# jkk-research/urban_road_filter

Measured on NVIDIA H100. Metric: scans_per_sec, higher is better.
Workload: dtype f32/f64

## Files before the change

### urban_road_filter_b200/csrc/urf_kernels.cuh

```cuda
#pragma once
#include <type_traits>

#include "urf_device.cuh"
#include "urf_logic.cuh"
#include "urf_lomuto.cuh"
#include "urf_stdsort.cuh"
#include "urf_workspace.cuh"

namespace urf {

__constant__ float c_beam_d[kSectKeys];
__constant__ float c_beam_o[kSectKeys];
__constant__ unsigned char c_beam_yx[kSectKeys];

__device__ __forceinline__ int lane_id() { return threadIdx.x & 31; }
__device__ __forceinline__ unsigned scan_base(int b, int S) { return (unsigned)b * point_slice((unsigned)S); }

template <int N, class T>
__device__ __forceinline__ void warp_inclusive_sum(T (&x)[N]) {
#pragma unroll
  for (int d = 1; d < 32; d <<= 1) {
    T u[N];
#pragma unroll
    for (int i = 0; i < N; i++) u[i] = __shfl_up_sync(0xffffffffu, x[i], d);
// ... 181 lines not shown
        buf.sect[g] = (short)sec;
      }
      const unsigned peers = __match_any_sync(0xffffffffu, sec);
      if (sec >= 0 && lane_id() == __ffs(peers) - 1) atomicAdd(&s_scnt[sec], __popc(peers));
    }
#pragma unroll
    for (int j = 0; j < kPtsPerThread; ++j) cur[j] = nxt[j];
  }
  roi = __reduce_add_sync(0xffffffffu, roi);
  if (lane_id() == 0 && roi) atomicAdd(&s_roi, roi);
  __syncthreads();
  unsigned* fi = buf.firstidx + (size_t)b * kElevSlice;
  for (int e = threadIdx.x; e <= kElevBins; e += kPtsThreads) {
    const unsigned v = s_first[e];
    if (v != 0xffffffffu) atomicMin(&fi[e], v);
  }
  for (int s = threadIdx.x; s < kSectKeys; s += kPtsThreads)
    if (s_scnt[s]) atomicAdd(&buf.tab[b].sect_cnt[s], s_scnt[s]);
  if (threadIdx.x == 0 && s_roi) atomicAdd(&buf.out[b].n_roi, s_roi);
}

__device__ void register_exact_cta(const float* __restrict__ alpha, int n, float interval, int channels, float* s_vis,
                                   float* s_reg, int* s_idx, int* out_m) {
  int m = 0, vis = 0, i_last = -1;
  bool frozen = false;
  while (m < channels) {
    int local = 0x7fffffff;
    for (int i = i_last + 1 + threadIdx.x; i < n; i += blockDim.x) {
      const float a = alpha[i];
      if (a < 0.0f) continue;
      bool cov = false;
      for (int t = 0; t < vis; t++) {
        if (fabsf(__fsub_rn(s_vis[t], a)) <= interval) { cov = true; break; }
      }
      if (!cov) { local = i; break; }
    }
    const int istar = CtaGroup::min(local);
    if (istar == 0x7fffffff) break;
    const float a = alpha[istar];
    if (threadIdx.x == 0) { s_reg[m] = a; s_idx[m] = istar; if (!frozen && a != 0.0f) s_vis[vis] = a; }
    if (!frozen) { if (a == 0.0f) frozen = true; else vis++; }
    m++;
    i_last = istar;
    __syncthreads();
  }
  *out_m = m;
}

__device__ void publish_rings_cta(ScanTab& tab, ScanOut& out, unsigned short* lut, float interval, const float* s_reg,
                                  const int* s_idx, int m, unsigned long long* s_keys, float* s_sorted) {
  for (int t = threadIdx.x; t < kRingKeys; t += blockDim.x)
    s_keys[t] = t < m ? (((unsigned long long)fbits(s_reg[t]) << 32) | (unsigned)s_idx[t]) : ~0ull;
  __syncthreads();
  group_bitonic<CtaGroup>(s_keys, kRingKeys);
  for (int t = threadIdx.x; t < kRingKeys; t += blockDim.x) {
    if (t < m) {
      const float a = bitsf((unsigned)(s_keys[t] >> 32));
      s_sorted[t] = a;
      tab.angle[t] = a;
      tab.regidx[t] = (int)(unsigned)s_keys[t];
      tab.regorder[t] = s_idx[t];
    } else { s_sorted[t] = 0.f; tab.angle[t] = 0.f; tab.regidx[t] = 0x7fffffff; tab.regorder[t] = 0x7fffffff; }
  }
  if (threadIdx.x == 0) out.n_rings = m;
  __syncthreads();
  for (int e = threadIdx.x; e <= kElevBins; e += blockDim.x) lut[e] = (unsigned short)ring_lut_entry(s_sorted, m, interval, e);
}

__global__ void __launch_bounds__(256) k_register(DevBuffers buf, DevParams prm, int S) {
  const int b = blockIdx.x;
  const int n = buf.n[b];
  ScanOut& out = buf.out[b];
  ScanTab& tab = buf.tab[b];
  const float* alpha = buf.alpha_v + (size_t)b * point_slice(S);
  __shared__ unsigned s_cand[kMaxCand];
  __shared__ float s_calpha[kMaxCand];
  __shared__ float s_vis[kRingKeys];
  __shared__ float s_reg[kRingKeys];
  __shared__ float s_sorted[kRingKeys];
  __shared__ int s_idx[kRingKeys];
  __shared__ unsigned long long s_keys[kRingKeys];
  __shared__ int s_cnt, s_m;
  if (out.n_roi < 30) {
    if (threadIdx.x == 0) out.n_rings = 0;
    return;
  }
  bool exact = prm.force_exact || (out.flags & F_ZERO_ALPHA);
  if (!exact) {
    if (threadIdx.x == 0) s_cnt = 0;
    __syncthreads();
    const unsigned* fi = buf.firstidx + (size_t)b * kElevSlice;
    for (int t = threadIdx.x; t <= kElevBins; t += blockDim.x) {
      const unsigned v = fi[t];
      if (v != 0xffffffffu) { int s = atomicAdd(&s_cnt, 1); if (s < kMaxCand) s_cand[s] = v; }
    }
    __syncthreads();
    const int cnt = s_cnt;
    if (cnt > kMaxCand) exact = true;
    else {
      const int npad = next_pow2(cnt < 2 ? 2 : cnt);
      for (int t = cnt + threadIdx.x; t < npad; t += blockDim.x) s_cand[t] = 0xffffffffu;
      __syncthreads();
      group_bitonic<CtaGroup>(s_cand, npad);
      for (int t = threadIdx.x; t < cnt; t += blockDim.x) s_calpha[t] = alpha[s_cand[t]];
      __syncthreads();
      if (threadIdx.x < 32) {
        int m = 0;
        for (int c = 0; c < cnt && m < prm.channels; c++) {
          const float a = s_calpha[c];
          bool cov = false;
          for (int t = lane_id(); t < m; t += 32)
            if (fabsf(__fsub_rn(s_reg[t], a)) <= prm.interval) cov = true;
          cov = __any_sync(0xffffffffu, cov);
          if (!cov) {
            if (lane_id() == 0) { s_reg[m] = a; s_idx[m] = (int)s_cand[c]; }
            m++;
            __syncwarp();
          }
        }
        if (lane_id() == 0) s_m = m;
      }
      __syncthreads();
    }
  }
  if (exact) {
    int m;
    register_exact_cta(alpha, n, prm.interval, prm.channels, s_vis, s_reg, s_idx, &m);
    if (threadIdx.x == 0) { s_m = m; atomicOr(&out.flags, F_EXACT_REG); }
    __syncthreads();
  }
  publish_rings_cta(tab, out, buf.lut + (size_t)b * kElevSlice, prm.interval, s_reg, s_idx, s_m, s_keys, s_sorted);
}

__device__ __forceinline__ bool assign_chunk(const DevBuffers& buf, const DevParams& prm, int b, int S, int T, int chunk, int n, bool live,
                                             bool verify, const float* s_angle, const int* s_regidx, const int* regorder, int R,
                                             const unsigned short* __restrict__ lut, unsigned* cnt, int lane) {
  bool violation = false;
  constexpr int H = 8;
  static_assert((kChunk / 32) % H == 0, "chunk iterations come in groups of H");
#pragma unroll 1
  for (int h0 = 0; h0 < kChunk / 32; h0 += H) {
    float av[H];
    unsigned short start[H];
#pragma unroll
    for (int u = 0; u < H; u++) {
      const int i = chunk * kChunk + (h0 + u) * 32 + lane;
      av[u] = i < n ? buf.alpha_v[scan_base(b, S) + (unsigned)i] : -1.0f;
    }
#pragma unroll
    for (int u = 0; u < H; u++) start[u] = (live && av[u] >= 0.0f) ? lut[elev_bin(av[u])] : (unsigned short)0;
#pragma unroll
    for (int u = 0; u < H; u++) {
      const int i = chunk * kChunk + (h0 + u) * 32 + lane;
      int ring = -1;
      if (i < n) {
        const float a = av[u];
        const bool kept = live && a >= 0.0f;
        if (kept) {
          int lo;
          ring = assign_ring_from(s_angle, R, a, prm.interval, start[u], &lo);
          if (verify && registration_violation(s_angle, s_regidx, regorder, R, prm.channels, prm.interval, a, i, lo)) violation = true;
        }
        buf.ringid[scan_base(b, S) + (unsigned)i] = kept ? (short)ring : (short)-2;
      }
      const int ring0 = __shfl_sync(0xffffffffu, ring, 0);
      if (__all_sync(0xffffffffu, ring == ring0)) { if (lane == 0 && ring0 >= 0) atomicAdd(&cnt[ring0], 32u); }
      else if (ring >= 0) atomicAdd(&cnt[ring], 1u);
    }
  }
  __syncwarp();
  const int C = prm.channels;
  unsigned* row = buf.hist + ((size_t)b * chunk_rows(T) + chunk) * C;
  for (int t = lane; t < C; t += 32) row[t] = cnt[t];
  return violation;
}

__global__ void __launch_bounds__(kWarpsPerBlock * 32) k_assign(DevBuffers buf, DevParams prm, int S, int T) {
  const int b = blockIdx.y;
  ScanOut& out = buf.out[b];
  const int flags = out.flags;
  const int n = buf.n[b];
  const int warp = threadIdx.x >> 5, lane = lane_id();
  const int chunk = blockIdx.x * kWarpsPerBlock + warp;
  __shared__ float s_angle[kRingKeys];
  __shared__ int s_regidx[kRingKeys];
  __shared__ unsigned s_cnt[kWarpsPerBlock][kRingKeys];
  ScanTab& tab = buf.tab[b];
  const int R = out.n_rings;
  for (int t = threadIdx.x; t < kRingKeys; t += blockDim.x) { s_angle[t] = tab.angle[t]; s_regidx[t] = tab.regidx[t]; }
  for (int t = lane; t < kRingKeys; t += 32) s_cnt[warp][t] = 0;
  __syncthreads();
  if (chunk * kChunk >= n) return;
  const bool violation = assign_chunk(buf, prm, b, S, T, chunk, n, out.n_roi >= 30, !(flags & F_EXACT_REG), s_angle, s_regidx, tab.regorder, R,
                                      buf.lut + (size_t)b * kElevSlice, s_cnt[warp], lane);
  if (__any_sync(0xffffffffu, violation) && lane == 0) atomicOr(&out.flags, F_SPEC_VIOLATION);
}

constexpr int kScanOffThreads = 512, kScanOffWarps = kScanOffThreads / 32;
constexpr int kScanOffBatch = 16;
static_assert(kRingKeys < kScanOffThreads && kSectKeys <= kScanOffThreads, "one ring_start entry and one sector per thread");
__global__ void __launch_bounds__(kScanOffThreads, 2) k_scan_offsets(DevBuffers buf, DevParams prm, int S, int T) {
  __shared__ unsigned s_part[kScanOffWarps][kRingKeys];
  __shared__ unsigned s_base[kRingKeys];
  const int b = blockIdx.x;
  const int n = buf.n[b];
  const int C = prm.channels;
  const int rows = (n + kChunk - 1) / kChunk;
  const int warp = threadIdx.x >> 5, lane = lane_id();
  {
    ScanOut& out = buf.out[b];
    const int flags = out.flags;
    if ((flags & F_SPEC_VIOLATION) && !(flags & F_EXACT_REG)) {
      __shared__ float s_vis[kRingKeys], s_reg[kRingKeys], s_sorted[kRingKeys];
      __shared__ int s_idx[kRingKeys];
      __shared__ unsigned long long s_keys[kRingKeys];
      __shared__ int s_m;
      int m;
      register_exact_cta(buf.alpha_v + (size_t)b * point_slice(S), n, prm.interval, prm.channels, s_vis, s_reg, s_idx, &m);
      if (threadIdx.x == 0) s_m = m;
      __syncthreads();
      const unsigned short* lut = buf.lut + (size_t)b * kElevSlice;
      publish_rings_cta(buf.tab[b], out, buf.lut + (size_t)b * kElevSlice, prm.interval, s_reg, s_idx, s_m, s_keys, s_sorted);
      __syncthreads();
      const int R = s_m;
      for (int c0 = 0; c0 < rows; c0 += kScanOffWarps) {
        for (int t = lane; t < kRingKeys; t += 32) s_part[warp][t] = 0;
        __syncwarp();
        if (c0 + warp < rows) assign_chunk(buf, prm, b, S, T, c0 + warp, n, true, false, s_sorted, nullptr, nullptr, R, lut, s_part[warp], lane);
        __syncwarp();
      }
      if (threadIdx.x == 0) out.flags = flags | F_EXACT_REG;
      __syncthreads();
    }
  }
  ScanTab& tab = buf.tab[b];
  const unsigned scnt = threadIdx.x < kSectKeys ? (unsigned)tab.sect_cnt[threadIdx.x] : 0u;
  const int rpw = (rows + kScanOffWarps - 1) / kScanOffWarps;
  const int r0 = min(rows, warp * rpw), r1 = min(rows, (warp + 1) * rpw);
  unsigned* hist = buf.hist + (size_t)b * chunk_rows(T) * C;
  for (int key = lane; key < C; key += 32) {
    unsigned s = 0;
    for (int r = r0; r < r1; r += kScanOffBatch) {
      unsigned v[kScanOffBatch];
#pragma unroll
      for (int u = 0; u < kScanOffBatch; u++) v[u] = r + u < r1 ? hist[(size_t)(r + u) * C + key] : 0u;
#pragma unroll
      for (int u = 0; u < kScanOffBatch; u++) s += v[u];
    }
    s_part[warp][key] = s;
  }
  __syncthreads();
  unsigned rtot = 0;
  if (threadIdx.x < C)
    for (int w = 0; w < kScanOffWarps; w++) { const unsigned v = s_part[w][threadIdx.x]; s_part[w][threadIdx.x] = rtot; rtot += v; }
  unsigned x[2] = {rtot, scnt}, all[2];
  CtaGroup::exclusive_sum(x, all);
  const unsigned xr = x[0], xs = x[1], all_r = all[0], all_s = all[1];
  ScanOut& o = buf.out[b];
  if (threadIdx.x < C) s_base[threadIdx.x] = xr;
  if (threadIdx.x <= kRingKeys) o.ring_start[threadIdx.x] = (int)(threadIdx.x < C ? xr : all_r);
  if (threadIdx.x < kSectKeys) { tab.sect_start[threadIdx.x] = (int)xs; tab.sect_cur[threadIdx.x] = (int)xs; }
  if (threadIdx.x == 0) { o.n_order = (int)all_r; tab.sect_start[kSectKeys] = (int)all_s; }
  __syncthreads();
  for (int key = lane; key < C; key += 32) {
    unsigned run = s_base[key] + s_part[warp][key];
    for (int r = r0; r < r1; r += kScanOffBatch) {
      unsigned v[kScanOffBatch];
#pragma unroll
      for (int u = 0; u < kScanOffBatch; u++) v[u] = r + u < r1 ? hist[(size_t)(r + u) * C + key] : 0u;
#pragma unroll
      for (int u = 0; u < kScanOffBatch; u++)
        if (r + u < r1) { hist[(size_t)(r + u) * C + key] = run; run += v[u]; }
    }
  }
}

__device__ __forceinline__ void mbar_init(unsigned long long* bar, unsigned count) {
  asm volatile("mbarrier.init.shared::cta.b64 [%0], %1;\n" ::"r"((unsigned)__cvta_generic_to_shared(bar)), "r"(count) : "memory");
  asm volatile("fence.proxy.async.shared::cta;\n" ::: "memory");
}
__device__ __forceinline__ void bulk_copy_g2s(void* dst, const void* src, unsigned bytes, unsigned long long* bar) {
  const unsigned d = (unsigned)__cvta_generic_to_shared(dst), m = (unsigned)__cvta_generic_to_shared(bar);
  asm volatile("mbarrier.arrive.expect_tx.shared::cta.b64 _, [%0], %1;\n" ::"r"(m), "r"(bytes) : "memory");
  asm volatile("cp.async.bulk.shared::cluster.global.mbarrier::complete_tx::bytes [%0], [%1], %2, [%3];\n"
               ::"r"(d), "l"(src), "r"(bytes), "r"(m) : "memory");
}
__device__ __forceinline__ void mbar_wait(unsigned long long* bar, unsigned phase) {
  const unsigned m = (unsigned)__cvta_generic_to_shared(bar);
  unsigned done;
  do {
    asm volatile("{\n .reg .pred p;\n mbarrier.try_wait.parity.shared::cta.b64 p, [%1], %2;\n selp.u32 %0, 1, 0, p;\n}\n"
                 : "=r"(done) : "r"(m), "r"(phase) : "memory");
  } while (!done);
}
constexpr int kScatterWarps = 4;
constexpr size_t kScatterSmem = (size_t)kScatterWarps * kChunk * sizeof(float4);
__global__ void __launch_bounds__(kScatterWarps * 32, 4) k_scatter(DevBuffers buf, DevParams prm, int S, int T) {
  const int b = blockIdx.y;
  const int n = buf.n[b];
  const int warp = threadIdx.x >> 5, lane = lane_id();
  const int chunk = blockIdx.x * kScatterWarps + warp;
  extern __shared__ float4 s_tiles[];
  __shared__ unsigned long long s_bar[kScatterWarps];
  __shared__ unsigned s_delta[kScatterWarps][kChunk];
  __shared__ unsigned s_lcnt[kScatterWarps][kRingKeys];
  __shared__ unsigned short s_perm[kScatterWarps][kChunk];
  __shared__ int s_scnt[kSectKeys], s_sbase[kSectKeys];
  const float4* tile = s_tiles + warp * kChunk;
  unsigned* delta = s_delta[warp];
  unsigned* lcnt = s_lcnt[warp];
  unsigned short* perm = s_perm[warp];
  ScanTab& tab = buf.tab[b];
  const bool live = chunk * kChunk < n;
  const unsigned* row = buf.hist + ((size_t)b * chunk_rows(T) + chunk) * prm.channels;
  const unsigned gb = scan_base(b, S), g0 = gb + (unsigned)chunk * kChunk;
  if (live && lane == 0) {
    mbar_init(&s_bar[warp], 1);
    bulk_copy_g2s(s_tiles + warp * kChunk, buf.in + g0, (unsigned)min(kChunk, n - chunk * kChunk) * sizeof(float4), &s_bar[warp]);
  }
  for (int t = threadIdx.x; t < kSectKeys; t += blockDim.x) s_scnt[t] = 0;
  for (int t = lane; t < kRingKeys; t += 32) lcnt[t] = 0;
  __syncthreads();
  const unsigned lt = (1u << lane) - 1u;
  unsigned packed[kChunk / 32];
  unsigned spack[kChunk / 32];
  if (live) {
    constexpr int GRP = kChunk / 32;
#pragma unroll
    for (int h = 0; h < kChunk / 32 / GRP; h++) {
      short rr[GRP], ss[GRP];
#pragma unroll
      for (int u = 0; u < GRP; u++) {
        const int li = (h * GRP + u) * 32 + lane;
        const bool in = chunk * kChunk + li < n;
        rr[u] = in ? buf.ringid[g0 + li] : (short)-1;
        ss[u] = in ? buf.sect[g0 + li] : (short)-1;
      }
#pragma unroll
      for (int u = 0; u < GRP; u++) {
        const int it = h * GRP + u;
        const int sec = ss[u];
        const int sec0 = __shfl_sync(0xffffffffu, sec, 0);
        int srank = 0;
        if (__all_sync(0xffffffffu, sec == sec0)) {
          int sb = 0;
          if (lane == 0 && sec0 >= 0) sb = atomicAdd(&s_scnt[sec0], 32);
          srank = __shfl_sync(0xffffffffu, sb, 0) + lane;
        } else if (sec >= 0) srank = atomicAdd(&s_scnt[sec], 1);
        spack[it] = sec >= 0 ? (((unsigned)(sec + 1) << 16) | (unsigned)srank) : 0u;
        const int ring = rr[u];
        const int rprev = __shfl_up_sync(0xffffffffu, ring, 1), ring0 = __shfl_sync(0xffffffffu, ring, 0);
        unsigned peers;
        if (__all_sync(0xffffffffu, ring == ring0)) peers = 0xffffffffu;
        else if (__all_sync(0xffffffffu, lane == 0 || ring > rprev) || __all_sync(0xffffffffu, lane == 0 || ring < rprev)) peers = 1u << lane;
        else peers = __match_any_sync(0xffffffffu, ring);
        const int leader = __ffs(peers) - 1;
        unsigned rb = 0;
        if (ring >= 0 && lane == leader) rb = atomicAdd(&lcnt[ring], (unsigned)__popc(peers));
        rb = __shfl_sync(0xffffffffu, rb, leader);
        packed[it] = ring >= 0 ? (((unsigned)(ring + 1) << 16) | (rb + __popc(peers & lt))) : 0u;
      }
    }
  }
  __syncthreads();
  for (int t = threadIdx.x; t < kSectKeys; t += blockDim.x) {
    const int c = s_scnt[t];
    s_sbase[t] = c > 0 ? atomicAdd(&tab.sect_cur[t], c) : 0;
  }
  int total = 0;
  if (live) {
    {
      unsigned v[kRingKeys / 32], sum = 0;
#pragma unroll
      for (int j = 0; j < kRingKeys / 32; j++) { v[j] = lcnt[lane * (kRingKeys / 32) + j]; sum += v[j]; }
      unsigned inc[1] = {sum};
      warp_inclusive_sum(inc);
      unsigned run = inc[0] - sum;
      __syncwarp();
#pragma unroll
      for (int j = 0; j < kRingKeys / 32; j++) { lcnt[lane * (kRingKeys / 32) + j] = run; run += v[j]; }
    }
    __syncwarp();
#pragma unroll
    for (int it = 0; it < kChunk / 32; it++) {
      const unsigned pk = packed[it];
      if (pk) {
        const int ring = (int)(pk >> 16) - 1;
        const unsigned lstart = lcnt[ring];
        const int slot = lstart + (pk & 0xffffu);
        perm[slot] = (unsigned short)(it * 32 + lane);
        delta[slot] = __ldg(&row[ring]) - lstart;
      }
      total += __popc(__ballot_sync(0xffffffffu, pk != 0));
    }
    __syncwarp();
    mbar_wait(&s_bar[warp], 0);
    for (int t = lane; t < total; t += 32) {
      const int li = perm[t];
      const float4 p = tile[li];
      const unsigned dst = gb + delta[t] + (unsigned)t;
      buf.bpt[dst] = make_float4(p.x, p.y, p.z, __int_as_float(chunk * kChunk + li));
      if (prm.want_order) buf.baz[dst] = make_uint2(fbits(buf.az[g0 + li]), (unsigned)(chunk * kChunk + li));
    }
  }
  __syncthreads();
  if (live) {
#pragma unroll
    for (int it = 0; it < kChunk / 32; it++) {
      const unsigned sp = spack[it];
      if (sp) {
        const int sec = (int)(sp >> 16) - 1;
        const int li = it * 32 + lane;
        const float4 p = tile[li];
        const unsigned dst = gb + (unsigned)(s_sbase[sec] + (int)(sp & 0xffffu));
        buf.sr[dst] = star_radius(p.x, p.y);
        buf.sz[dst] = p.z;
        buf.sidx[dst] = (unsigned)(chunk * kChunk + li);
      }
    }
  }
}

constexpr int kWarpCap = 1024, kCtaCap = 8192;
constexpr int kNetCap = 512;
constexpr unsigned kSslIndex = 0x80000000u;

struct SectorRecs {
  const DevBuffers& buf;
  unsigned o;
  unsigned at;
  __device__ __forceinline__ const float* r() const { return buf.sr + o; }
  __device__ __forceinline__ unsigned key(int e) const { return fbits(buf.sr[o + (unsigned)e]); }
  __device__ __forceinline__ void put(int e, unsigned k, unsigned slot) const {
    buf.ssrz[at + (unsigned)e] = make_float2(bitsf(k), buf.sz[o + slot]);
    buf.ssl[at + (unsigned)e] = slot;
  }
};
__device__ __forceinline__ SectorRecs sector_recs(const DevBuffers& buf, int b, int S, int base, int at = 0) {
  const unsigned o = scan_base(b, S) + (unsigned)base;
  return SectorRecs{buf, o, o + (unsigned)at};
}
__device__ __forceinline__ int star_input_index(const DevBuffers& buf, unsigned o, int e) {
  const unsigned l = buf.ssl[o + (unsigned)e];
  return (l & kSslIndex) ? (int)(l & ~kSslIndex) : (int)buf.sidx[o + l];
}

template <int EPL, int WARPS, bool LIST = false, bool STAGED = false>
__device__ __forceinline__ bool bitonic_sector(const SectorRecs& d, int n, int tid, unsigned* s_xk, unsigned* s_xe) {
  constexpr int THREADS = WARPS * 32;
  const int lane = tid & 31;
  unsigned key[EPL], el[EPL];
#pragma unroll
  for (int r = 0; r < EPL; r++) {
    const int e = tid * EPL + r;
    key[r] = 0xffffffffu; el[r] = 0u;
    if (e < n) {
      if (LIST) { key[r] = s_xk[e]; el[r] = (STAGED && s_xe == nullptr) ? (unsigned)e : s_xe[e]; }
      else { key[r] = d.key(e); el[r] = (unsigned)e; }
    }
  }
  auto intra = [&](int k_over_epl, auto kc) {
    constexpr int K = decltype(kc)::value;
#pragma unroll
    for (int j = (K > 0 ? K : EPL) >> 1; j > 0; j >>= 1) {
#pragma unroll
      for (int r = 0; r < EPL; r++) {
        if ((r & j) == 0) {
          const bool asc = K > 0 ? ((r & K) == 0) : ((tid & k_over_epl) == 0);
          const bool sw = (key[r] > key[r | j]) == asc;
          const unsigned ka = sw ? key[r | j] : key[r], kb = sw ? key[r] : key[r | j];
          const unsigned ea = sw ? el[r | j] : el[r], eb = sw ? el[r] : el[r | j];
          key[r] = ka; key[r | j] = kb; el[r] = ea; el[r | j] = eb;
        }
      }
    }
  };
  if (EPL > 2) intra(0, std::integral_constant<int, 2>());
  if (EPL > 4) intra(0, std::integral_constant<int, 4>());
  if (EPL > 8) intra(0, std::integral_constant<int, 8>());
  if (EPL > 16) intra(0, std::integral_constant<int, 16>());
  for (int ke = 1; ke <= THREADS; ke <<= 1) {
    for (int tj = ke >> 1; tj > 0; tj >>= 1) {
      const bool keep_min = ((tid & tj) == 0) == ((tid & ke) == 0);
      if (tj < 32) {
#pragma unroll
        for (int r = 0; r < EPL; r++) {
          const unsigned o = __shfl_xor_sync(0xffffffffu, key[r], tj);
          const unsigned oe = __shfl_xor_sync(0xffffffffu, el[r], tj);
          const bool take = (o < key[r]) == keep_min;
          key[r] = take ? o : key[r];
          el[r] = take ? oe : el[r];
        }
      } else {
        __syncthreads();
#pragma unroll
        for (int r = 0; r < EPL; r++) { s_xk[r * THREADS + tid] = key[r]; s_xe[r * THREADS + tid] = el[r]; }
        __syncthreads();
#pragma unroll
        for (int r = 0; r < EPL; r++) {
          const unsigned o = s_xk[r * THREADS + (tid ^ tj)], oe = s_xe[r * THREADS + (tid ^ tj)];
          const bool take = (o < key[r]) == keep_min;
          key[r] = take ? o : key[r];
          el[r] = take ? oe : el[r];
        }
      }
    }
    intra(ke, std::integral_constant<int, 0>());
  }
  unsigned prev0 = __shfl_up_sync(0xffffffffu, key[EPL - 1], 1);
  if (WARPS > 1) {
    __syncthreads();
    if (lane == 31) s_xk[tid >> 5] = key[EPL - 1];
    __syncthreads();
    if (lane == 0 && tid > 0) prev0 = s_xk[(tid >> 5) - 1];
  }
  bool tie = false;
  if constexpr (STAGED) {
    static_assert(!STAGED || (WARPS == 1 && LIST && EPL <= 16), "STAGED: single-warp list sorts of up to 16 elements per lane");
#pragma unroll
    for (int r = 0; r < EPL; r++) {
      const int e = tid * EPL + r;
      const unsigned prev = r > 0 ? key[r - 1] : prev0;
      if (e < n && e > 0 && prev == key[r]) tie = true;
    }
    static_assert(!STAGED || 32 * EPL <= kNetCap, "STAGED: the keys go kNetCap words above the slots");
    constexpr int TPW = 32 / EPL;
    __syncwarp();
#pragma unroll
    for (int r = 0; r < EPL; r++) {
      const int w = tid * EPL + (r ^ ((tid / TPW) & (EPL - 1)));
      s_xk[w] = el[r];
      s_xk[kNetCap + w] = key[r];
    }
    __syncwarp();
#pragma unroll
    for (int r = 0; r < EPL; r++) {
      const int e = r * 32 + tid, t = e / EPL;
      const int w = t * EPL + ((e & (EPL - 1)) ^ ((t / TPW) & (EPL - 1)));
      if (e < n) d.put(e, s_xk[kNetCap + w], s_xk[w]);
    }
    __syncwarp();
  } else {
#pragma unroll
    for (int r = 0; r < EPL; r++) {
      const int e = tid * EPL + r;
      const unsigned prev = r > 0 ? key[r - 1] : prev0;
      if (e < n) {
        d.put(e, key[r], el[r]);
        if (e > 0 && prev == key[r]) tie = true;
      }
    }
  }
  return tie;
}

__device__ __forceinline__ bool near_prefix(int m, int n) { return m >= 32 && 4 * m <= 3 * n; }

template <int EPL>
__device__ __forceinline__ int select_near(unsigned* kb, int n, int lane, int pivot_rank) {
  const unsigned mine = kb[(int)(((unsigned)lane * (unsigned)n) >> 5)];
  unsigned key[EPL];
#pragma unroll
  for (int r = 0; r < EPL; r++) {
    const int e = r * 32 + lane;
    key[r] = e < n ? kb[e] : 0xffffffffu;
  }
  int rank = 0;
#pragma unroll
  for (int j = 0; j < 32; j++) { const unsigned o = __shfl_sync(0xffffffffu, mine, j); rank += (o < mine) || (o == mine && j < lane); }
  const unsigned pivot = __shfl_sync(0xffffffffu, mine, __ffs(__ballot_sync(0xffffffffu, rank == pivot_rank)) - 1);
  int m = 0;
#pragma unroll
  for (int r = 0; r < EPL; r++) m += __popc(__ballot_sync(0xffffffffu, key[r] < pivot));
  if (!near_prefix(m, n) || m > kNetCap) return m;
  __syncwarp();
  const unsigned lt = (1u << lane) - 1u;
  int pos0 = 0;
#pragma unroll
  for (int r = 0; r < EPL; r++) {
    const bool sel = key[r] < pivot;
    const unsigned bs = __ballot_sync(0xffffffffu, sel);
    const int pos = pos0 + __popc(bs & lt);
    if (sel) { kb[pos] = key[r]; kb[kNetCap + pos] = (unsigned)(r * 32 + lane); }
    pos0 += __popc(bs);
  }
  __syncwarp();
  return m;
}

template <int EPL>
__device__ __forceinline__ int select_far(const float* __restrict__ sr, int n, int lane, unsigned* s_pk, unsigned* s_pe, unsigned kmax) {
  unsigned key[EPL];
#pragma unroll
  for (int r = 0; r < EPL; r++) {
    const int e = r * 32 + lane;
    key[r] = e < n ? fbits(sr[e]) : 0u;
  }
  const unsigned lt = (1u << lane) - 1u;
  int m = 0;
#pragma unroll
  for (int r = 0; r < EPL; r++) {
    const bool sel = key[r] > kmax;
    const unsigned bs = __ballot_sync(0xffffffffu, sel);
    if (sel) { const int pos = m + __popc(bs & lt); s_pk[pos] = key[r]; s_pe[pos] = (unsigned)(r * 32 + lane); }
    m += __popc(bs);
  }
  __syncwarp();
  return m;
}

constexpr int kPrefixMin = 128;

__device__ __forceinline__ void cp_async4(unsigned* s, const float* g) {
  asm volatile("cp.async.ca.shared.global [%0], [%1], 4;\n" ::"r"((unsigned)__cvta_generic_to_shared(s)), "l"(g) : "memory");
}
__device__ __forceinline__ void cp_async16(unsigned* s, const float* g) {
  asm volatile("cp.async.cg.shared.global [%0], [%1], 16;\n" ::"r"((unsigned)__cvta_generic_to_shared(s)), "l"(g) : "memory");
}
__device__ __forceinline__ void cp_async_commit() { asm volatile("cp.async.commit_group;\n" ::: "memory"); }
template <int N>
__device__ __forceinline__ void cp_async_wait() { asm volatile("cp.async.wait_group %0;\n" ::"n"(N) : "memory"); }

__device__ __forceinline__ void star_sort_sector(const DevBuffers& buf, const DevParams& prm, int S, int b, int s, int base, int n,
                                                 unsigned* kb, int lane) {
  ScanTab& tab = buf.tab[b];
  if (lane == 0) tab.sorted_len[s] = n;
  if (n <= 0) return;
  const SectorRecs d = sector_recs(buf, b, S, base);
  if (n == 1) { if (lane == 0) d.put(0, d.key(0), 0u); return; }
  if (n > kWarpCap) {
    if (lane == 0) {
      if (n <= kCtaCap) tab.biglist[atomicAdd(&tab.nbig, 1)] = (unsigned short)s;
      else tab.slowlist[atomicAdd(&tab.nslow, 1)] = (unsigned short)s;
    }
    return;
  }
  int m = 0;
  if (prm.star_prefix && n > kPrefixMin) {
    if (n <= 256) m = select_near<8>(kb, n, lane, prm.star_pivot);
    else if (n <= 512) m = select_near<16>(kb, n, lane, prm.star_pivot);
    else m = select_near<32>(kb, n, lane, prm.star_pivot);
  }
  const bool near = near_prefix(m, n);
  const int len = near ? m : n;
  if (len > kNetCap) {
    if (lane == 0) tab.biglist[atomicAdd(&tab.nbig, 1)] = (unsigned short)s;
    return;
  }
  unsigned* pe = near ? kb + kNetCap : nullptr;
  bool tie;
  if (len <= 128) tie = bitonic_sector<4, 1, true, true>(d, len, lane, kb, pe);
  else if (len <= 256) tie = bitonic_sector<8, 1, true, true>(d, len, lane, kb, pe);
  else tie = bitonic_sector<16, 1, true, true>(d, len, lane, kb, pe);
  if (near && lane == 0) tab.sorted_len[s] = m;
  if (__any_sync(0xffffffffu, tie) && lane == 0) tab.slowlist[atomicAdd(&tab.nslow, 1)] = (unsigned short)s;
}

constexpr int kSortWarps = 8;
constexpr int kStage = kWarpCap + 4;
constexpr size_t kStarSortSmem = (size_t)kSortWarps * 2 * kStage * sizeof(unsigned);
__global__ void __launch_bounds__(kSortWarps * 32, 3) k_star_sort(DevBuffers buf, DevParams prm, int S, int B) {
  extern __shared__ unsigned s_dyn[];
  const int lane = lane_id(), warp = __shfl_sync(0xffffffffu, (int)threadIdx.x >> 5, 0);
  unsigned* const stage = s_dyn + (size_t)warp * 2 * kStage;
  const int Q = B * kSectKeys, W = gridDim.x * kSortWarps;
  auto offsets = [&](int q, int& base, int& n) {
    int v = 0;
    if (q < Q && lane < 2) { const int b = q / kSectKeys; v = buf.tab[b].sect_start[q - b * kSectKeys + lane]; }
    base = __shfl_sync(0xffffffffu, v, 0);
    n = __shfl_sync(0xffffffffu, v, 1) - base;
  };
  auto radii = [&](int q, int base) { return buf.sr + (size_t)(q / kSectKeys) * S + base; };
  auto key_word = [](const float* g) { return (int)((reinterpret_cast<uintptr_t>(g) >> 2) & 3); };
  auto stage_keys = [&](int q, int base, int n, unsigned* st) {
    if (q < Q && n > 1 && n <= kWarpCap) {
      const float* g = radii(q, base);
      const int off = key_word(g);
      unsigned* kb = st + off;
      const int h = min(n, (4 - off) & 3);
      const int nv = (n - h) >> 2, t0 = h + 4 * nv;
      for (int v = lane; v < nv; v += 32) cp_async16(kb + h + 4 * v, g + h + 4 * v);
      if (lane < h + (n - t0)) { const int e = lane < h ? lane : t0 + (lane - h); cp_async4(kb + e, g + e); }
    }
    cp_async_commit();
  };
  int q = blockIdx.x * kSortWarps + warp;
  int base, n, nbase, nn;
  offsets(q, base, n);
  stage_keys(q, base, n, stage);
  offsets(q + W, nbase, nn);
  for (int it = 0; q < Q; q += W, it ^= 1) {
    stage_keys(q + W, nbase, nn, stage + (it ^ 1) * kStage);
    int base2, n2;
    offsets(q + 2 * W, base2, n2);
    cp_async_wait<1>();
    __syncwarp();
    const int b = q / kSectKeys;
    star_sort_sector(buf, prm, S, b, q - b * kSectKeys, base, n, stage + it * kStage + key_word(radii(q, base)), lane);
    __syncwarp();
    base = nbase; n = nn; nbase = base2; nn = n2;
  }
  cp_async_wait<0>();
}

template <class G>
__device__ void slow_sort_sector(const DevBuffers& buf, int b, int S, int base, int n, unsigned long long* s_keys, int cap) {
  const size_t o = (size_t)b * point_slice(S) + base;
  const int npad = next_pow2(n < 2 ? 2 : n);
// ... 1022 lines not shown
```

Measured before the change: 88130.

## Merge per-warp ring bucketing into CTA-wide scatter for contiguous writes

Replaces the per-warp local ring offsets and scatter with a CTA-wide exclusive scan over all warps' ring counts, so points from the four chunks in a block that share a ring are laid out contiguously and the write-out loop runs across the whole block. Each ring's global base is loaded once per CTA instead of once per point. The aim is longer contiguous global write runs and less redundant histogram reading. The cost is an extra CTA-wide scan and barrier, and it assumes the histogram row at the block's first chunk gives the right base for all the chunks in the block.

New measurement: 89300, median of 6. 1.01x the previous value.

```diff
diff --git a/urban_road_filter_b200/csrc/urf_kernels.cuh b/urban_road_filter_b200/csrc/urf_kernels.cuh
--- a/urban_road_filter_b200/csrc/urf_kernels.cuh
+++ b/urban_road_filter_b200/csrc/urf_kernels.cuh
@@ -507,17 +507,17 @@
   const int chunk = blockIdx.x * kScatterWarps + warp;
   extern __shared__ float4 s_tiles[];
   __shared__ unsigned long long s_bar[kScatterWarps];
-  __shared__ unsigned s_delta[kScatterWarps][kChunk];
+  __shared__ unsigned s_delta[kScatterWarps * kChunk];
   __shared__ unsigned s_lcnt[kScatterWarps][kRingKeys];
-  __shared__ unsigned short s_perm[kScatterWarps][kChunk];
+  __shared__ unsigned short s_perm[kScatterWarps * kChunk];
+  __shared__ unsigned s_rbase[kRingKeys];
   __shared__ int s_scnt[kSectKeys], s_sbase[kSectKeys];
   const float4* tile = s_tiles + warp * kChunk;
-  unsigned* delta = s_delta[warp];
   unsigned* lcnt = s_lcnt[warp];
-  unsigned short* perm = s_perm[warp];
   ScanTab& tab = buf.tab[b];
   const bool live = chunk * kChunk < n;
-  const unsigned* row = buf.hist + ((size_t)b * chunk_rows(T) + chunk) * prm.channels;
+  const int c0 = blockIdx.x * kScatterWarps;
+  const unsigned* row0 = buf.hist + ((size_t)b * chunk_rows(T) + c0) * prm.channels;
   const unsigned gb = scan_base(b, S), g0 = gb + (unsigned)chunk * kChunk;
   if (live && lane == 0) {
     mbar_init(&s_bar[warp], 1);
@@ -572,43 +572,51 @@
     const int c = s_scnt[t];
     s_sbase[t] = c > 0 ? atomicAdd(&tab.sect_cur[t], c) : 0;
   }
-  int total = 0;
+  constexpr int kRpt = kRingKeys / (kScatterWarps * 32);
+  static_assert(kRpt * kScatterWarps * 32 == kRingKeys, "whole rings per thread");
+  unsigned total;
+  {
+    unsigned cnt[kRpt][kScatterWarps], tot[kRpt], x[1] = {0u}, all[1];
+#pragma unroll
+    for (int j = 0; j < kRpt; j++) {
+      tot[j] = 0;
+#pragma unroll
+      for (int w = 0; w < kScatterWarps; w++) { cnt[j][w] = s_lcnt[w][threadIdx.x * kRpt + j]; tot[j] += cnt[j][w]; }
+      x[0] += tot[j];
+    }
+    CtaGroup::exclusive_sum(x, all);
+    total = all[0];
+    unsigned run = x[0];
+#pragma unroll
+    for (int j = 0; j < kRpt; j++) {
+      const int r = threadIdx.x * kRpt + j;
+      s_rbase[r] = (tot[j] > 0 ? __ldg(&row0[r]) : 0u) - run;
+#pragma unroll
+      for (int w = 0; w < kScatterWarps; w++) { s_lcnt[w][r] = run; run += cnt[j][w]; }
+    }
+  }
+  __syncthreads();
   if (live) {
-    {
-      unsigned v[kRingKeys / 32], sum = 0;
-#pragma unroll
-      for (int j = 0; j < kRingKeys / 32; j++) { v[j] = lcnt[lane * (kRingKeys / 32) + j]; sum += v[j]; }
-      unsigned inc[1] = {sum};
-      warp_inclusive_sum(inc);
-      unsigned run = inc[0] - sum;
-      __syncwarp();
-#pragma unroll
-      for (int j = 0; j < kRingKeys / 32; j++) { lcnt[lane * (kRingKeys / 32) + j] = run; run += v[j]; }
-    }
-    __syncwarp();
 #pragma unroll
     for (int it = 0; it < kChunk / 32; it++) {
       const unsigned pk = packed[it];
       if (pk) {
         const int ring = (int)(pk >> 16) - 1;
-        const unsigned lstart = lcnt[ring];
-        const int slot = lstart + (pk & 0xffffu);
-        perm[slot] = (unsigned short)(it * 32 + lane);
-        delta[slot] = __ldg(&row[ring]) - lstart;
-      }
-      total += __popc(__ballot_sync(0xffffffffu, pk != 0));
-    }
-    __syncwarp();
+        const int slot = lcnt[ring] + (pk & 0xffffu);
+        s_perm[slot] = (unsigned short)(warp * kChunk + it * 32 + lane);
+        s_delta[slot] = s_rbase[ring];
+      }
+    }
     mbar_wait(&s_bar[warp], 0);
-    for (int t = lane; t < total; t += 32) {
-      const int li = perm[t];
-      const float4 p = tile[li];
-      const unsigned dst = gb + delta[t] + (unsigned)t;
-      buf.bpt[dst] = make_float4(p.x, p.y, p.z, __int_as_float(chunk * kChunk + li));
-      if (prm.want_order) buf.baz[dst] = make_uint2(fbits(buf.az[g0 + li]), (unsigned)(chunk * kChunk + li));
-    }
-  }
-  __syncthreads();
+  }
+  __syncthreads();
+  for (int t = threadIdx.x; t < (int)total; t += blockDim.x) {
+    const int li = s_perm[t];
+    const float4 p = s_tiles[li];
+    const unsigned dst = gb + s_delta[t] + (unsigned)t;
+    buf.bpt[dst] = make_float4(p.x, p.y, p.z, __int_as_float(c0 * kChunk + li));
+    if (prm.want_order) buf.baz[dst] = make_uint2(fbits(buf.az[gb + (unsigned)c0 * kChunk + li]), (unsigned)(c0 * kChunk + li));
+  }
   if (live) {
 #pragma unroll
     for (int it = 0; it < kChunk / 32; it++) {
```
